# TtesseractT/Synthetic-Audio-Detection

Hardware: AMD Instinct MI355X
Metric: 4s@32kHz segments/sec end-to-end (mel+ResNet+ensemble), 1/2/4/8 MI355X (higher is better)
Workload: dtype bf16; 1 GPU; end-to-end inference: B int16 4 s segments resident in HBM -> mel front end -> ResNet-18@512x512 -> 6 binary heads -> merge (+RCCL all-gather of logits); heads=6, distinct_backbones=1, micro_batch=2048, parallelism=dp1, frontend_overlapped=True

## Files before the change

synthetic-audio-detection_amd/csrc/l2conv.hip:

```cpp
#include "common.hpp"
#include "igemm.hpp"
#include "kernels.hpp"
#include "rwconv.hpp"

namespace sad {

namespace l2c {
constexpr int NW = 4;
constexpr int PW = 18, PR = PW * PW;
constexpr int NDP = (PR + 7) / 8;
constexpr int PATCH = NDP * 1024;
constexpr int ROWB = PW * 128;
constexpr int QP = (NDP + NW - 1) / NW;
constexpr int RESB = 256 * 256;
constexpr int NRP = RESB / 1024 / NW;
constexpr int NDS = 256 * 128 / 1024 / NW;
constexpr int OFF_RES = 2 * PATCH;
constexpr int SMEM_RES = OFF_RES + RESB;
constexpr int NS = 36;
constexpr int NSC = 18;
constexpr int DQ = 4;
constexpr int WV = 8;
constexpr int BAD = 0x7FFFFFF0;
constexpr uint64_t KEY = 0xd92dad912240ull;
constexpr int TABB = NW * QP * 256;
constexpr int TAIL = 512 + TABB;
constexpr int ESH = 27;
static_assert(SMEM_RES + TAIL <= 160 * 1024, "LDS budget");
static_assert(PATCH % 128 == 0 && OFF_RES % 256 == 0, "buffer offsets commute with the chunk XORs");
}

__device__ __forceinline__ int l2c_key(int x) { return (int)((l2c::KEY >> (3 * x)) & 7); }

template <bool RES, bool DS, bool X3, bool ST, bool AB, typename E = u16>
__device__ __forceinline__ void l2conv_body(const BlockConvArgs& a) {
  static_assert(!is_f16_v<E> || (!X3 && !ST && !AB), "fp16: the plain inference forms");
  f16_kernel_entry<E>();
  static_assert(!(RES && DS) && !(X3 && DS), "one shortcut form");
  static_assert(!ST || (!RES && !DS && !X3), "statistics: the plain bf16 form");
  static_assert(!AB || (!X3 && !ST), "ablations: the bf16 forms");
  using namespace l2c;
  constexpr int TP = X3 ? 8 : 16;
  constexpr int UPT = 2 * TP;
  constexpr int NUC = 9 * UPT;
  constexpr int PDIV = X3 ? 8 : 16;
  constexpr int DQ = X3 ? 8 : l2c::DQ;
  constexpr int OFF_B = RES || DS ? SMEM_RES : OFF_RES;
  constexpr int OFF_T = OFF_B + 512;
  extern __shared__ __attribute__((aligned(256))) char smem[];
  const int tid = threadIdx.x, lane = tid & 63;
  const int wave = __builtin_amdgcn_readfirstlane(tid >> 6);
  const int fr = lane & 15, fg = lane >> 4;
  const int ab = AB ? a.ablate : 0;
  const int cw = X3 ? (wave & 1) * 32 : wave * 32;
  const int r0w = X3 ? (wave >> 1) * 8 : 0;
  const int w = xcd_remap(blockIdx.x, gridDim.x);
  const int tiles_x = a.W / 16, tiles_img = tiles_x * (a.H / 16);
  const int tiles_p = a.N * tiles_img;
  const int tp_begin = (int)((int64_t)w * tiles_p / gridDim.x), tp_end = (int)((int64_t)(w + 1) * tiles_p / gridDim.x);
  if (tp_begin >= tp_end) {
    if constexpr (ST) a.st_part[(int64_t)w * 256 + tid] = 0.f;
    return;
  }

  l1b_v4 rx = {(unsigned)(uintptr_t)a.in0, (unsigned)((uintptr_t)a.in0 >> 32) & 0xFFFFu, (unsigned)a.in0_bytes, 0x00020000u};
  asm volatile("" : "+s"(rx));
  const void* const rrp = RES ? (const void*)a.res : (const void*)a.in1;
  l1b_v4 rr = {(unsigned)(uintptr_t)rrp, (unsigned)((uintptr_t)rrp >> 32) & 0xFFFFu,
               (unsigned)(RES ? a.res_bytes : a.in1_bytes), 0x00020000u};
  if constexpr (RES || DS) asm volatile("" : "+s"(rr));
  const __amdgpu_buffer_rsrc_t ro =
      __builtin_amdgcn_make_buffer_rsrc((void*)a.out, (short)0, (int)a.out_bytes, 0x00020000);
  const unsigned lds0 = (unsigned)(uintptr_t)(__attribute__((address_space(3))) char*)smem;
  const int ps = (int)a.in0_pstride * 2;
  const int pso = (int)a.out_pstride * 2;
  const int pss = RES ? (int)a.res_pstride * 2 : DS ? a.ss1 * (int)a.in1_pstride * 2 : 0;
  const int srow = RES ? a.W * pss : DS ? a.ss1 * a.W1 * (int)a.in1_pstride * 2 : 0;
  const int orow = a.W * pso;

  struct TileO {
    int base, oy0, ox0, sbase, obase;
  };
  auto tile_o = [&](int t) __attribute__((always_inline)) {
    const int b = t / tiles_img, rem = t - b * tiles_img;
    const int ty = rem / tiles_x;
    TileO o;
    o.oy0 = ty * 16;
    o.ox0 = (rem - ty * tiles_x) * 16;
    o.base = ((b * a.H + o.oy0) * a.W + o.ox0) * ps;
    o.obase = ((b * a.H + o.oy0) * a.W + o.ox0) * pso;
    o.sbase = RES  ? ((b * a.H + o.oy0) * a.W + o.ox0) * pss
              : DS ? ((b * a.H1 + o.oy0 * a.ss1) * a.W1 + o.ox0 * a.ss1) * (int)(a.in1_pstride * 2)
                   : 0;
    return o;
  };
  const int wrap_i = 15 * a.W * ps, wrap_o = 15 * orow, wrap_s = 16 * srow - a.W * pss;
  auto tile_step = [&](const TileO& o) __attribute__((always_inline)) {
    TileO n;
    n.ox0 = o.ox0 + 16;
    n.oy0 = o.oy0;
    n.base = o.base + 16 * ps;
    n.obase = o.obase + 16 * pso;
    n.sbase = o.sbase + 16 * pss;
    if (n.ox0 == a.W) {
      n.ox0 = 0;
      n.oy0 += 16;
      n.base += wrap_i;
      n.obase += wrap_o;
      n.sbase += wrap_s;
      if (n.oy0 == a.H) n.oy0 = 0;
    }
    return n;
  };

  const int TA = (int)lds0 + OFF_T + (wave * (QP * 64) + lane) * 4;
  auto piece_entry = [&](int k) __attribute__((always_inline)) {
    const int r = 8 * (wave + NW * k) + (lane >> 3);
    const int Y = (r * 3641) >> 16, X = r - PW * Y;
    const int edge = (r >= PR ? 1 : 0) | (Y == 0 ? 2 : 0) | (Y == PW - 1 ? 4 : 0) | (X == 0 ? 8 : 0) | (X == PW - 1 ? 16 : 0);
    const unsigned off = (unsigned)((Y * a.W + X) * ps + (((lane & 7) ^ l2c_key(X)) << 4)) >> 4;
    return (int)(((unsigned)edge << ESH) | (off & ((1u << ESH) - 1)));
  };
  auto patch_base = [&](const TileO& o) __attribute__((always_inline)) { return o.base - (a.W + 1) * ps; };
  auto patch_mask = [&](const TileO& o) __attribute__((always_inline)) {
    return (int)((unsigned)(1 | (o.oy0 == 0 ? 2 : 0) | (o.oy0 + 16 == a.H ? 4 : 0) | (o.ox0 == 0 ? 8 : 0) |
                            (o.ox0 + 16 == a.W ? 16 : 0))
                 << ESH);
  };
  const unsigned dstw = __builtin_amdgcn_readfirstlane(lds0 + wave * 1024);
  auto issue_piece = [&](auto kc, auto cc, int e, int pbase, int pmask) __attribute__((always_inline)) {
    constexpr int k = decltype(kc)::value, c = decltype(cc)::value;
    if constexpr (NW * k + NW - 1 >= NDP)
      if (wave + NW * k >= NDP) return;
    l1b_dma16<c * PATCH + k * NW * 1024>(rx, (e & pmask) ? BAD : pbase + (int)((unsigned)e << 4), dstw);
  };
  const int pxr = 4 * wave + (lane >> 4);
  const int RV = pxr * pss + (((lane & 15) ^ pxr) << 4);
  auto issue_res = [&](auto kc, const TileO& o) __attribute__((always_inline)) {
    constexpr int k = decltype(kc)::value;
    l1b_dma16<OFF_RES + k * NW * 1024>(rr, RV + (o.sbase + k * srow), dstw);
  };
  const int pxd = 8 * (wave & 1) + (lane >> 3);
  const int DV = (wave >> 1) * srow + pxd * pss + (((lane & 7) ^ ((pxd >> 1) & 7)) << 4);
  auto issue_ds = [&](auto kc, const TileO& o) __attribute__((always_inline)) {
    constexpr int k = decltype(kc)::value;
    l1b_dma16<OFF_RES + k * NW * 1024>(rr, DV + (o.sbase + 2 * k * srow), dstw);
  };
  l1b_v4 wds[2][2];
  if constexpr (DS) {
#pragma unroll
    for (int i = 0; i < 2; ++i)
#pragma unroll
      for (int h = 0; h < 2; ++h)
        wds[i][h] = *(const l1b_v4*)((const u16*)a.wt + (size_t)(cw + 16 * i + fr) * a.wt_ld + 9 * 128 + (fg + 4 * h) * 8);
  }

  l1b_v4 wr[2][NS];
#pragma unroll
  for (int i = 0; i < 2; ++i)
#pragma unroll
    for (int s = 0; s < NS; ++s) {
      const int c = s / NSC, tap = (s % NSC) >> 1, h = s & 1;
      wr[i][s] = *(const l1b_v4*)((const u16*)a.wt + (size_t)(cw + 16 * i + fr) * a.wt_ld + tap * 128 + c * 64 +
                                  (fg + 4 * h) * 8);
    }
  if (tid < (X3 ? 16 : 32)) *(float4*)(smem + OFF_B + 16 * tid) = *(const float4*)(a.bias + 4 * tid);
  TileO ocur = tile_o(tp_begin);
  l1b_for<QP>([&](auto kc) __attribute__((always_inline)) {
    constexpr int k = decltype(kc)::value;
    const int e = piece_entry(k);
    l1b_st<int>(TA + 256 * k, e);
    issue_piece(kc, std::integral_constant<int, 0>{}, e, patch_base(ocur), patch_mask(ocur));
  });

  int I2[3];
#pragma unroll
  for (int kx = 0; kx < 3; ++kx)
    I2[kx] = (int)lds0 + r0w * ROWB + (fr + kx) * 128 + ((fg ^ l2c_key(fr + kx)) << 4);
  const int BA = (int)lds0 + OFF_B + (cw + fg * 4) * 4;
  const int OV = ((r0w + (fg & 1)) * a.W + fr) * pso + ((X3 ? 64 * (cw >> 5) : cw) + (fg >> 1) * 8) * 2;
  const int RB = (int)lds0 + OFF_RES + (r0w * 16 + fr) * 256 + ((((X3 ? 8 * (cw >> 5) : cw >> 3) + (fg >> 1)) ^ fr) << 4) +
                 (fg & 1) * 8;
  const int DD = (int)lds0 + OFF_RES + fr * 128 + ((fg ^ ((fr >> 1) & 7)) << 4);
  const int rl = a.relu ? 0 : (int)0x80008000u;
  const bool relu = a.relu;

  asm volatile("s_waitcnt vmcnt(0)" ::: "memory");
  __syncthreads();
  f32x4 acc[2][TP];
#pragma unroll
  for (int i = 0; i < 2; ++i) {
    const f32x4 b0 = l1b_ld<f32x4>(BA + 64 * i);
#pragma unroll
    for (int j = 0; j < TP; ++j) acc[i][j] = b0;
  }

  float st_s[2][4] = {}, st_q[2][4] = {};
  for (int t = tp_begin; t < tp_end; ++t) {
    const TileO ostep = tile_step(ocur);
    const TileO onext = t + 1 < tp_end ? ostep : ocur;
    const TileO o = ocur;
    const int pb1 = patch_base(o) + 128, pm1 = patch_mask(o);
    const int pb0n = patch_base(onext), pm0n = patch_mask(onext);

    l1b_for<2>([&](auto cc) __attribute__((always_inline)) {
      constexpr int c = decltype(cc)::value;
      if constexpr (c == 0)
        asm volatile("s_waitcnt vmcnt(16)" ::: "memory");
      else
        asm volatile("s_waitcnt vmcnt(0)" ::: "memory");
      __builtin_amdgcn_s_barrier();
      asm volatile("" ::: "memory");
      int pe = l1b_ld<int>(TA);
      int I2c[3][2];
#pragma unroll
      for (int kx = 0; kx < 3; ++kx) {
        I2c[kx][0] = I2[kx] + c * PATCH;
        I2c[kx][1] = I2c[kx][0] ^ 64;
      }
      auto rd = [&](auto uc) __attribute__((always_inline)) -> l1b_v4 {
        constexpr int u = decltype(uc)::value;
        constexpr int tap = u / UPT, ky = tap / 3, kx = tap % 3;
        constexpr int j = X3 ? (u % UPT) / 2 : u % 16, h = X3 ? u % 2 : (u % UPT) / 16;
        return l1b_ld<l1b_v4>(I2c[kx][h] + (j + ky) * ROWB);
      };
      l1b_v4 bq[DQ];
      l1b_for<DQ>([&](auto uc) __attribute__((always_inline)) { bq[decltype(uc)::value] = rd(uc); });
      l1b_for<NUC>([&](auto uc) __attribute__((always_inline)) {
        constexpr int u = decltype(uc)::value;
        constexpr int tap = u / UPT;
        constexpr int j = X3 ? (u % UPT) / 2 : u % 16, h = X3 ? u % 2 : (u % UPT) / 16;
        constexpr int s = c * NSC + 2 * tap + h;
        constexpr int s_hi = c * NSC + 2 * tap, s_lo = s_hi + 1;
        const l1b_v4 bf = bq[u % DQ];
        if constexpr (u + DQ < NUC) bq[u % DQ] = rd(std::integral_constant<int, u + DQ>{});
        if constexpr (u % PDIV == 0 && u / PDIV < QP) {
          constexpr int k = u / PDIV;
          if (!(ab & 32))
            issue_piece(std::integral_constant<int, k>{}, std::integral_constant<int, c ^ 1>{}, pe, c == 0 ? pb1 : pb0n,
                        c == 0 ? pm1 : pm0n);
          if constexpr (k + 1 < QP) pe = l1b_ld<int>(TA + 256 * (k + 1));
        }
        if constexpr (RES && c == 0 && u % PDIV == PDIV / 2 && u / PDIV < NRP)
          issue_res(std::integral_constant<int, u / PDIV>{}, o);
        if constexpr (DS && c == 0 && u % 32 == 8 && u / 32 < NDS) issue_ds(std::integral_constant<int, u / 32>{}, o);
        auto mm = [&](auto ic, auto sc) __attribute__((always_inline)) {
          constexpr int i = decltype(ic)::value, ss = decltype(sc)::value;
          if constexpr (i == 1 && ss >= NS - WV)
            l1b_mfma_v<E>(acc[i][j], wr[i][ss], bf);
          else
            l1b_mfma_a<E>(acc[i][j], wr[i][ss], bf);
        };
        if constexpr (!X3) {
          mm(std::integral_constant<int, 0>{}, std::integral_constant<int, s>{});
          mm(std::integral_constant<int, 1>{}, std::integral_constant<int, s>{});
        } else if constexpr (u == NUC - 2) {
          const l1b_v4 xl = bq[(u + 1) % DQ];
          static_assert(j == TP - 1 && h == 0, "last fragment");
          if constexpr (s_hi >= NS - WV)
            asm volatile(
                "v_mfma_f32_16x16x32_bf16 %0, %2, %6, %0\n\t"
                "v_mfma_f32_16x16x32_bf16 %1, %3, %6, %1\n\t"
                "v_mfma_f32_16x16x32_bf16 %0, %4, %6, %0\n\t"
                "v_mfma_f32_16x16x32_bf16 %1, %5, %6, %1\n\t"
                "v_mfma_f32_16x16x32_bf16 %0, %2, %7, %0\n\t"
                "v_mfma_f32_16x16x32_bf16 %1, %3, %7, %1\n\t"
                "s_nop 11"
                : "+v"(acc[0][j]), "+v"(acc[1][j])
                : "a"(wr[0][s_hi]), "v"(wr[1][s_hi]), "a"(wr[0][s_lo]), "v"(wr[1][s_lo]), "v"(bf), "v"(xl));
          else
            asm volatile(
                "v_mfma_f32_16x16x32_bf16 %0, %2, %6, %0\n\t"
                "v_mfma_f32_16x16x32_bf16 %1, %3, %6, %1\n\t"
                "v_mfma_f32_16x16x32_bf16 %0, %4, %6, %0\n\t"
                "v_mfma_f32_16x16x32_bf16 %1, %5, %6, %1\n\t"
                "v_mfma_f32_16x16x32_bf16 %0, %2, %7, %0\n\t"
                "v_mfma_f32_16x16x32_bf16 %1, %3, %7, %1\n\t"
                "s_nop 11"
                : "+v"(acc[0][j]), "+v"(acc[1][j])
                : "a"(wr[0][s_hi]), "a"(wr[1][s_hi]), "a"(wr[0][s_lo]), "a"(wr[1][s_lo]), "v"(bf), "v"(xl));
        } else if constexpr (u == NUC - 1) {
        } else if constexpr (h == 0) {
          mm(std::integral_constant<int, 0>{}, std::integral_constant<int, s_hi>{});
          mm(std::integral_constant<int, 1>{}, std::integral_constant<int, s_hi>{});
          mm(std::integral_constant<int, 0>{}, std::integral_constant<int, s_lo>{});
          mm(std::integral_constant<int, 1>{}, std::integral_constant<int, s_lo>{});
        } else {
          mm(std::integral_constant<int, 0>{}, std::integral_constant<int, s_hi>{});
          mm(std::integral_constant<int, 1>{}, std::integral_constant<int, s_hi>{});
        }
      });
    });
    if constexpr (DS) {
      constexpr int DQD = 8;
      const int DD1 = DD ^ 64;
      auto rdd = [&](auto uc) __attribute__((always_inline)) -> l1b_v4 {
        constexpr int u = decltype(uc)::value;
        return l1b_ld<l1b_v4>((u / 16 ? DD1 : DD) + (u % 16) * 16 * 128);
      };
      l1b_v4 bd[DQD];
      l1b_for<DQD>([&](auto uc) __attribute__((always_inline)) { bd[decltype(uc)::value] = rdd(uc); });
      l1b_for<32>([&](auto uc) __attribute__((always_inline)) {
        constexpr int u = decltype(uc)::value, h = u / 16, j = u % 16;
        const l1b_v4 bf = bd[u % DQD];
        if constexpr (u + DQD < 32) bd[u % DQD] = rdd(std::integral_constant<int, u + DQD>{});
        l1b_mfma_v<E>(acc[0][j], wds[0][h], bf);
        l1b_mfma_v<E>(acc[1][j], wds[1][h], bf);
      });
    }
    __builtin_amdgcn_sched_barrier(0);
    asm volatile("s_nop 11" ::: "memory");
    __builtin_amdgcn_sched_barrier(0);
    f32x4 bv[2];
#pragma unroll
    for (int i = 0; i < 2; ++i) bv[i] = l1b_ld<f32x4>(BA + 64 * i);

#pragma unroll
    for (int j = 0; j < TP; j += 2) {
      const int osj = o.obase + j * orow;
#pragma unroll
      for (int i = 0; i < 2; ++i) {
        f32x4 v0 = acc[i][j], v1 = acc[i][j + 1];
        const int rbi = i ? RB ^ 32 : RB;
        if constexpr (X3) {
          if constexpr (RES) {
            const l1b_v2 h0 = l1b_ld<l1b_v2>(rbi + j * 4096);
            const l1b_v2 l0 = l1b_ld<l1b_v2>((rbi ^ 64) + j * 4096);
            const l1b_v2 h1 = l1b_ld<l1b_v2>(rbi + (j + 1) * 4096);
            const l1b_v2 l1 = l1b_ld<l1b_v2>((rbi ^ 64) + (j + 1) * 4096);
            v0[0] += __uint_as_float(h0.x << 16) + __uint_as_float(l0.x << 16);
            v0[1] += __uint_as_float(h0.x & 0xFFFF0000u) + __uint_as_float(l0.x & 0xFFFF0000u);
            v0[2] += __uint_as_float(h0.y << 16) + __uint_as_float(l0.y << 16);
            v0[3] += __uint_as_float(h0.y & 0xFFFF0000u) + __uint_as_float(l0.y & 0xFFFF0000u);
            v1[0] += __uint_as_float(h1.x << 16) + __uint_as_float(l1.x << 16);
            v1[1] += __uint_as_float(h1.x & 0xFFFF0000u) + __uint_as_float(l1.x & 0xFFFF0000u);
            v1[2] += __uint_as_float(h1.y << 16) + __uint_as_float(l1.y << 16);
            v1[3] += __uint_as_float(h1.y & 0xFFFF0000u) + __uint_as_float(l1.y & 0xFFFF0000u);
          }
          if (relu)
#pragma unroll
            for (int r = 0; r < 4; ++r) {
              v0[r] = fmaxf(v0[r], 0.f);
              v1[r] = fmaxf(v1[r], 0.f);
            }
          uint32_t qh[4] = {l1b_pk(v0[0], v0[1]), l1b_pk(v0[2], v0[3]), l1b_pk(v1[0], v1[1]), l1b_pk(v1[2], v1[3])};
          const float vv[8] = {v0[0], v0[1], v0[2], v0[3], v1[0], v1[1], v1[2], v1[3]};
          uint32_t ql[4];
#pragma unroll
          for (int e = 0; e < 4; ++e)
            ql[e] = l1b_pk(vv[2 * e] - __uint_as_float(qh[e] << 16), vv[2 * e + 1] - __uint_as_float(qh[e] & 0xFFFF0000u));
#pragma unroll
          for (int e = 0; e < 2; ++e) {
            const auto rh = __builtin_amdgcn_permlane16_swap(qh[e], qh[e + 2], false, false);
            qh[e] = rh[0];
            qh[e + 2] = rh[1];
            const auto rl2 = __builtin_amdgcn_permlane16_swap(ql[e], ql[e + 2], false, false);
            ql[e] = rl2[0];
            ql[e + 2] = rl2[1];
          }
          __builtin_amdgcn_raw_buffer_store_b128((l1b_v4){qh[0], qh[1], qh[2], qh[3]}, ro, OV + 32 * i, osj, 0);
          __builtin_amdgcn_raw_buffer_store_b128((l1b_v4){ql[0], ql[1], ql[2], ql[3]}, ro, OV + 32 * i + 64, osj, 0);
          acc[i][j] = bv[i];
          acc[i][j + 1] = bv[i];
          continue;
        }
        if constexpr (RES) {
          const l1b_v2 r0 = l1b_ld<l1b_v2>(rbi + j * 4096);
          const l1b_v2 r1 = l1b_ld<l1b_v2>(rbi + (j + 1) * 4096);
          v0[0] += lo16<E>(r0.x);
          v0[1] += hi16<E>(r0.x);
          v0[2] += lo16<E>(r0.y);
          v0[3] += hi16<E>(r0.y);
          v1[0] += lo16<E>(r1.x);
          v1[1] += hi16<E>(r1.x);
          v1[2] += lo16<E>(r1.y);
          v1[3] += hi16<E>(r1.y);
        }
        if constexpr (ST) {
#pragma unroll
          for (int e = 0; e < 4; ++e) {
            st_s[i][e] += v0[e];
            st_s[i][e] += v1[e];
            st_q[i][e] = fmaf(v0[e], v0[e], st_q[i][e]);
            st_q[i][e] = fmaf(v1[e], v1[e], st_q[i][e]);
          }
        }
        uint32_t q[4] = {l1b_pk<E>(v0[0], v0[1]), l1b_pk<E>(v0[2], v0[3]), l1b_pk<E>(v1[0], v1[1]),
                         l1b_pk<E>(v1[2], v1[3])};
        if constexpr (!ST)
#pragma unroll
          for (int e = 0; e < 4; ++e) q[e] = l1b_relu2s(q[e], rl);
#pragma unroll
        for (int e = 0; e < 2; ++e) {
          const auto r = __builtin_amdgcn_permlane16_swap(q[e], q[e + 2], false, false);
          q[e] = r[0];
          q[e + 2] = r[1];
        }
        if (!(ab & 8)) __builtin_amdgcn_raw_buffer_store_b128((l1b_v4){q[0], q[1], q[2], q[3]}, ro, OV + 32 * i, osj, 0);
        acc[i][j] = bv[i];
        acc[i][j + 1] = bv[i];
      }
    }
    ocur = ostep;
  }
  if constexpr (ST) {
#pragma unroll
    for (int i = 0; i < 2; ++i)
#pragma unroll
      for (int e = 0; e < 4; ++e)
#pragma unroll
        for (int off = 1; off < 16; off <<= 1) {
          st_s[i][e] += __shfl_xor(st_s[i][e], off, 64);
          st_q[i][e] += __shfl_xor(st_q[i][e], off, 64);
        }
    if (fr == 0) {
#pragma unroll
      for (int i = 0; i < 2; ++i)
#pragma unroll
        for (int e = 0; e < 4; ++e) {
          const int c = cw + 16 * i + 4 * fg + e;
          a.st_part[(int64_t)w * 256 + c] = st_s[i][e];
          a.st_part[(int64_t)w * 256 + 128 + c] = st_q[i][e];
        }
    }
  }
  asm volatile("s_waitcnt vmcnt(0)" ::: "memory");
}

template <bool RES, bool DS, bool X3 = false, bool ST = false, typename E = u16>
__global__ __launch_bounds__(256, 1) void l2conv_kernel(BlockConvArgs a) {
  l2conv_body<RES, DS, X3, ST, false, E>(a);
}
template <bool RES, bool DS>
__global__ __launch_bounds__(256, 1) void l2conv_ablate_kernel(BlockConvArgs a) {
  l2conv_body<RES, DS, false, false, true>(a);
}

int launch_l2conv(const BlockConvArgs& a, hipStream_t s, bool x3, bool h16) {
  using namespace l2c;
  SAD_REQUIRE(a.KH == 3 && a.KW == 3 && a.stride == 1 && a.pad == 1 && !a.pool_out,
              "variant 41/42: 3x3/s1/p1, no pool");
  SAD_REQUIRE(!h16 || (!x3 && !a.st_part && !a.ablate), "variant 41 in fp16: the plain inference forms");
  SAD_REQUIRE(!a.st_part || (!x3 && !a.in1 && !a.res && !a.relu && a.st_rows),
              "variant 41 statistics: the plain bf16 raw conv (no shortcut / residual / ReLU), st_rows set");
  if (x3) {
    SAD_REQUIRE(!a.in1 && a.Cin == 128 && a.Cout == 64 && a.H % 16 == 0 && a.W % 16 == 0 && a.Ho == a.H &&
                    a.Wo == a.W && a.wt_ld >= 9 * 128 && a.wt_ld % 8 == 0 && a.in0_pstride % 64 == 0 &&
                    a.in0_pstride >= 128 && a.out_pstride % 64 == 0 && a.out_pstride >= 128 &&
                    (!a.res || (a.res_pstride % 64 == 0 && a.res_pstride >= 128)) && a.out,
                "variant 42: split-bf16 64 -> 64 logical 3x3/s1/p1 (layer1), 16 x 16 tiles");
    const int64_t tiles = (int64_t)a.N * (a.H / 16) * (a.W / 16);
    if (tiles == 0) return SAD_OK;
    const int64_t g = std::min<int64_t>(tiles, 256);
    BlockConvArgs b = a;
    b.out_bytes = ((int64_t)a.N * a.H * a.W - 1) * a.out_pstride * 2 + 256;
    SAD_REQUIRE(b.out_bytes < (1ll << 31) - 65536, "variant 42: output passes the 32-bit buffer range");
    static bool attr[2] = {false, false};
    const void* kfn = a.res ? (const void*)l2conv_kernel<true, false, true> : (const void*)l2conv_kernel<false, false, true>;
    const int smem = (a.res ? SMEM_RES : OFF_RES) + TAIL;
    if (!attr[a.res ? 1 : 0]) {
      SAD_CHECK_HIP(hipFuncSetAttribute(kfn, hipFuncAttributeMaxDynamicSharedMemorySize, smem));
      attr[a.res ? 1 : 0] = true;
    }
    if (a.res)
      hipLaunchKernelGGL((l2conv_kernel<true, false, true>), dim3((unsigned)g), dim3(256), smem, s, b);
    else
      hipLaunchKernelGGL((l2conv_kernel<false, false, true>), dim3((unsigned)g), dim3(256), smem, s, b);
    SAD_CHECK_HIP(hipGetLastError());
    return SAD_OK;
  }
  SAD_REQUIRE(!a.in1 || (!a.res && a.Cin1 == 64 && a.ss1 == 2 && a.H1 == 2 * a.H && a.W1 == 2 * a.W &&
                         a.in1_pstride % 8 == 0 && a.wt_ld >= 9 * 128 + 64),
              "variant 41: the shortcut is a 1x1/2 downsample of a 64-channel input at twice the size");
  SAD_REQUIRE(a.Cin == 128 && a.Cout == 128, "variant 41: Cin = Cout = 128");
  SAD_REQUIRE(a.H % 16 == 0 && a.W % 16 == 0 && a.Ho == a.H && a.Wo == a.W, "variant 41: image must tile by 16 x 16");
  SAD_REQUIRE(a.wt_ld >= 9 * 128 && a.wt_ld % 8 == 0, "variant 41: weight rows");
  SAD_REQUIRE(a.in0_pstride % 8 == 0 && a.out_pstride % 8 == 0 && (!a.res || a.res_pstride % 8 == 0) &&
                  a.in0_pstride >= 128 && a.out_pstride >= 128 && (!a.res || a.res_pstride >= 128),
              "variant 41: 16-B aligned pixel strides");
  SAD_REQUIRE(a.out, "null output");
  const int64_t tiles = (int64_t)a.N * (a.H / 16) * (a.W / 16);
  if (tiles == 0) return SAD_OK;
  const int64_t g = std::min<int64_t>(tiles, 256);
  BlockConvArgs b = a;
  b.out_bytes = ((int64_t)a.N * a.H * a.W - 1) * a.out_pstride * 2 + 256;
  SAD_REQUIRE(b.out_bytes < (1ll << 31) - 65536, "variant 41: output passes the 32-bit buffer range");
  auto go = [&](auto kern, int smem, bool& attr) {
    if (!attr) {
      SAD_CHECK_HIP(hipFuncSetAttribute((const void*)kern, hipFuncAttributeMaxDynamicSharedMemorySize, smem));
      attr = true;
    }
    hipLaunchKernelGGL(kern, dim3((unsigned)g), dim3(256), smem, s, b);
    return SAD_OK;
  };
  static bool attr[10] = {};
  int rc;
  if (h16) {
    rc = a.res   ? go(l2conv_kernel<true, false, false, false, f16>, SMEM_RES + TAIL, attr[7])
         : a.in1 ? go(l2conv_kernel<false, true, false, false, f16>, SMEM_RES + TAIL, attr[8])
                 : go(l2conv_kernel<false, false, false, false, f16>, OFF_RES + TAIL, attr[9]);
  } else if (a.st_part) {
    rc = go(l2conv_kernel<false, false, false, true>, OFF_RES + TAIL, attr[6]);
    if (rc == SAD_OK) *a.st_rows = (int)g;
  } else if (a.res) {
    rc = a.ablate ? go(l2conv_ablate_kernel<true, false>, SMEM_RES + TAIL, attr[3])
                  : go(l2conv_kernel<true, false>, SMEM_RES + TAIL, attr[0]);
  } else if (a.in1) {
    rc = a.ablate ? go(l2conv_ablate_kernel<false, true>, SMEM_RES + TAIL, attr[4])
                  : go(l2conv_kernel<false, true>, SMEM_RES + TAIL, attr[1]);
  } else {
    rc = a.ablate ? go(l2conv_ablate_kernel<false, false>, OFF_RES + TAIL, attr[5])
                  : go(l2conv_kernel<false, false>, OFF_RES + TAIL, attr[2]);
  }
  if (rc != SAD_OK) return rc;
  SAD_CHECK_HIP(hipGetLastError());
  return SAD_OK;
}

}
```

Measured before the change: 64500 segments/s.

## Interleave conv epilogue and downsample MFMAs into the second-half MAC loop

For the non-X3 layer-2 conv, the second chunk's MAC loop is reordered to finish row-pairs early. Each finished pair's epilogue (residual add, stats, pack, relu, permlane swap, store) is then interleaved into the following pair's MFMAs. The downsample 1x1 MFMAs are folded into the same schedule, and the bias is applied through the first MFMA's accumulator input instead of a separate reinit. The aim is to hide the serial epilogue tail behind matrix-core work, at the cost of more complex scheduling and possible extra register pressure.

```diff
diff --git a/synthetic-audio-detection_amd/csrc/l2conv.hip b/synthetic-audio-detection_amd/csrc/l2conv.hip
--- a/synthetic-audio-detection_amd/csrc/l2conv.hip
+++ b/synthetic-audio-detection_amd/csrc/l2conv.hip
@@ -19,6 +19,7 @@
 constexpr int SMEM_RES = OFF_RES + RESB;
 constexpr int NS = 36;
 constexpr int NSC = 18;
+constexpr int SA = 12;
 constexpr int DQ = 4;
 constexpr int WV = 8;
 constexpr int BAD = 0x7FFFFFF0;
@@ -31,6 +32,22 @@
 }
 
 __device__ __forceinline__ int l2c_key(int x) { return (int)((l2c::KEY >> (3 * x)) & 7); }
+
+struct L2Unit {
+  int tap, h, j;
+  bool ds;
+};
+template <bool X3, bool DS>
+constexpr L2Unit l2c_unit(int c, int u) {
+  using l2c::SA;
+  if (X3) return {u / 16, u % 2, (u % 16) / 2, false};
+  if (c == 0 || u < SA * 16) return {u / 32, (u % 32) / 16, u % 16, false};
+  const int nb2 = 2 * (l2c::NSC - SA), upp = nb2 + (DS ? 4 : 0);
+  const int p = (u - SA * 16) / upp, w = (u - SA * 16) % upp;
+  if (w >= nb2) return {0, (w - nb2) / 2, 2 * p + (w - nb2) % 2, true};
+  const int s = SA + w / 2;
+  return {s / 2, s % 2, 2 * p + w % 2, false};
+}
 
 template <bool RES, bool DS, bool X3, bool ST, bool AB, typename E = u16>
 __device__ __forceinline__ void l2conv_body(const BlockConvArgs& a) {
@@ -45,6 +62,15 @@
   constexpr int NUC = 9 * UPT;
   constexpr int PDIV = X3 ? 8 : 16;
   constexpr int DQ = X3 ? 8 : l2c::DQ;
+  constexpr bool FO = !X3;
+  constexpr int NB = NSC - SA;
+  constexpr int UPP = 2 * NB + (DS ? 4 : 0);
+  constexpr int NUA = SA * TP;
+  constexpr int NU1 = FO ? NUA + (TP / 2) * UPP : NUC;
+  constexpr int PD1 = FO ? (NUA / QP < PDIV ? NUA / QP : PDIV) : PDIV;
+  static_assert(!FO || (SA >= 1 && SA < NSC && PD1 >= 1 && PD1 * (QP - 1) < NUA), "phase A carries the 11 pieces");
+  constexpr int EW0 = RES ? 4 : 2, EST = (UPP - EW0) / 8;
+  static_assert(!FO || EST >= 1, "a pair's MFMAs cover the previous pair's epilogue parts");
   constexpr int OFF_B = RES || DS ? SMEM_RES : OFF_RES;
   constexpr int OFF_T = OFF_B + 512;
   extern __shared__ __attribute__((aligned(256))) char smem[];
@@ -188,11 +214,13 @@
   asm volatile("s_waitcnt vmcnt(0)" ::: "memory");
   __syncthreads();
   f32x4 acc[2][TP];
-#pragma unroll
-  for (int i = 0; i < 2; ++i) {
-    const f32x4 b0 = l1b_ld<f32x4>(BA + 64 * i);
-#pragma unroll
-    for (int j = 0; j < TP; ++j) acc[i][j] = b0;
+  if constexpr (!FO) {
+#pragma unroll
+    for (int i = 0; i < 2; ++i) {
+      const f32x4 b0 = l1b_ld<f32x4>(BA + 64 * i);
+#pragma unroll
+      for (int j = 0; j < TP; ++j) acc[i][j] = b0;
+    }
   }
 
   float st_s[2][4] = {}, st_q[2][4] = {};
@@ -202,6 +230,61 @@
     const TileO o = ocur;
     const int pb1 = patch_base(o) + 128, pm1 = patch_mask(o);
     const int pb0n = patch_base(onext), pm0n = patch_mask(onext);
+    f32x4 bv[2];
+    if constexpr (FO) {
+#pragma unroll
+      for (int i = 0; i < 2; ++i) bv[i] = l1b_ld<f32x4>(BA + 64 * i);
+    }
+
+    l1b_v2 er[2][2];
+    uint32_t eq[4];
+    auto epi = [&](auto jc, auto pc) __attribute__((always_inline)) {
+      constexpr int j = decltype(jc)::value, part = decltype(pc)::value;
+      if constexpr (part == 0) {
+        if constexpr (RES) {
+#pragma unroll
+          for (int i = 0; i < 2; ++i)
+#pragma unroll
+            for (int k = 0; k < 2; ++k) er[i][k] = l1b_ld<l1b_v2>((i ? RB ^ 32 : RB) + (j + k) * 4096);
+        }
+      } else {
+        constexpr int i = (part - 1) / 4, k = (part - 1) % 4;
+        if constexpr (k < 2) {
+          f32x4& v = acc[i][j + k];
+          if constexpr (RES) {
+            v[0] += lo16<E>(er[i][k].x);
+            v[1] += hi16<E>(er[i][k].x);
+            v[2] += lo16<E>(er[i][k].y);
+            v[3] += hi16<E>(er[i][k].y);
+          }
+          if constexpr (ST) {
+#pragma unroll
+            for (int e = 0; e < 4; ++e) {
+              st_s[i][e] += v[e];
+              st_q[i][e] = fmaf(v[e], v[e], st_q[i][e]);
+            }
+          }
+        } else if constexpr (k == 2) {
+          const f32x4 v0 = acc[i][j], v1 = acc[i][j + 1];
+          eq[0] = l1b_pk<E>(v0[0], v0[1]);
+          eq[1] = l1b_pk<E>(v0[2], v0[3]);
+          eq[2] = l1b_pk<E>(v1[0], v1[1]);
+          eq[3] = l1b_pk<E>(v1[2], v1[3]);
+          if constexpr (!ST)
+#pragma unroll
+            for (int e = 0; e < 4; ++e) eq[e] = l1b_relu2s(eq[e], rl);
+        } else {
+#pragma unroll
+          for (int e = 0; e < 2; ++e) {
+            const auto r = __builtin_amdgcn_permlane16_swap(eq[e], eq[e + 2], false, false);
+            eq[e] = r[0];
+            eq[e + 2] = r[1];
+          }
+          if (!(ab & 8))
+            __builtin_amdgcn_raw_buffer_store_b128((l1b_v4){eq[0], eq[1], eq[2], eq[3]}, ro, OV + 32 * i, o.obase + j * orow, 0);
+        }
+      }
+    };
 
     l1b_for<2>([&](auto cc) __attribute__((always_inline)) {
       constexpr int c = decltype(cc)::value;
@@ -218,24 +301,28 @@
         I2c[kx][0] = I2[kx] + c * PATCH;
         I2c[kx][1] = I2c[kx][0] ^ 64;
       }
+      constexpr int NU = c == 0 ? NUC : NU1, PD = c == 0 ? PDIV : PD1;
+      const int DD1 = DD ^ 64;
       auto rd = [&](auto uc) __attribute__((always_inline)) -> l1b_v4 {
-        constexpr int u = decltype(uc)::value;
-        constexpr int tap = u / UPT, ky = tap / 3, kx = tap % 3;
-        constexpr int j = X3 ? (u % UPT) / 2 : u % 16, h = X3 ? u % 2 : (u % UPT) / 16;
-        return l1b_ld<l1b_v4>(I2c[kx][h] + (j + ky) * ROWB);
+        constexpr L2Unit U = l2c_unit<X3, DS>(c, decltype(uc)::value);
+        constexpr int ky = U.tap / 3, kx = U.tap % 3;
+        if constexpr (U.ds)
+          return l1b_ld<l1b_v4>((U.h ? DD1 : DD) + U.j * 16 * 128);
+        else
+          return l1b_ld<l1b_v4>(I2c[kx][U.h] + (U.j + ky) * ROWB);
       };
       l1b_v4 bq[DQ];
       l1b_for<DQ>([&](auto uc) __attribute__((always_inline)) { bq[decltype(uc)::value] = rd(uc); });
-      l1b_for<NUC>([&](auto uc) __attribute__((always_inline)) {
+      l1b_for<NU>([&](auto uc) __attribute__((always_inline)) {
         constexpr int u = decltype(uc)::value;
-        constexpr int tap = u / UPT;
-        constexpr int j = X3 ? (u % UPT) / 2 : u % 16, h = X3 ? u % 2 : (u % UPT) / 16;
+        constexpr L2Unit U = l2c_unit<X3, DS>(c, u);
+        constexpr int tap = U.tap, j = U.j, h = U.h;
         constexpr int s = c * NSC + 2 * tap + h;
         constexpr int s_hi = c * NSC + 2 * tap, s_lo = s_hi + 1;
         const l1b_v4 bf = bq[u % DQ];
-        if constexpr (u + DQ < NUC) bq[u % DQ] = rd(std::integral_constant<int, u + DQ>{});
-        if constexpr (u % PDIV == 0 && u / PDIV < QP) {
-          constexpr int k = u / PDIV;
+        if constexpr (u + DQ < NU) bq[u % DQ] = rd(std::integral_constant<int, u + DQ>{});
+        if constexpr (u % PD == 0 && u / PD < QP) {
+          constexpr int k = u / PD;
           if (!(ab & 32))
             issue_piece(std::integral_constant<int, k>{}, std::integral_constant<int, c ^ 1>{}, pe, c == 0 ? pb1 : pb0n,
                         c == 0 ? pm1 : pm0n);
@@ -246,7 +333,11 @@
         if constexpr (DS && c == 0 && u % 32 == 8 && u / 32 < NDS) issue_ds(std::integral_constant<int, u / 32>{}, o);
         auto mm = [&](auto ic, auto sc) __attribute__((always_inline)) {
           constexpr int i = decltype(ic)::value, ss = decltype(sc)::value;
-          if constexpr (i == 1 && ss >= NS - WV)
+          if constexpr (FO && U.ds)
+            l1b_mfma_v<E>(acc[i][j], wds[i][h], bf);
+          else if constexpr (FO && ss == 0)
+            l1b_mfma_ac<E>(acc[i][j], wr[i][ss], bf, bv[i]);
+          else if constexpr (i == 1 && ss >= NS - WV)
             l1b_mfma_v<E>(acc[i][j], wr[i][ss], bf);
           else
             l1b_mfma_a<E>(acc[i][j], wr[i][ss], bf);
@@ -254,6 +345,15 @@
         if constexpr (!X3) {
           mm(std::integral_constant<int, 0>{}, std::integral_constant<int, s>{});
           mm(std::integral_constant<int, 1>{}, std::integral_constant<int, s>{});
+          if constexpr (c == 1 && u >= NUA + UPP) {
+            constexpr int w = (u - NUA) % UPP, jp = 2 * ((u - NUA) / UPP - 1);
+            constexpr int part = w == 0 ? 0 : w >= EW0 && (w - EW0) % EST == 0 && (w - EW0) / EST < 8 ? 1 + (w - EW0) / EST : -1;
+            if constexpr (part == 0 ? RES : part > 0 && (RES || ST || (part - 1) % 4 >= 2)) {
+              __builtin_amdgcn_sched_barrier(0);
+              epi(std::integral_constant<int, jp>{}, std::integral_constant<int, part>{});
+              __builtin_amdgcn_sched_barrier(0);
+            }
+          }
         } else if constexpr (u == NUC - 2) {
           const l1b_v4 xl = bq[(u + 1) % DQ];
           static_assert(j == TP - 1 && h == 0, "last fragment");
@@ -291,38 +391,22 @@
         }
       });
     });
-    if constexpr (DS) {
-      constexpr int DQD = 8;
-      const int DD1 = DD ^ 64;
-      auto rdd = [&](auto uc) __attribute__((always_inline)) -> l1b_v4 {
-        constexpr int u = decltype(uc)::value;
-        return l1b_ld<l1b_v4>((u / 16 ? DD1 : DD) + (u % 16) * 16 * 128);
-      };
-      l1b_v4 bd[DQD];
-      l1b_for<DQD>([&](auto uc) __attribute__((always_inline)) { bd[decltype(uc)::value] = rdd(uc); });
-      l1b_for<32>([&](auto uc) __attribute__((always_inline)) {
-        constexpr int u = decltype(uc)::value, h = u / 16, j = u % 16;
-        const l1b_v4 bf = bd[u % DQD];
-        if constexpr (u + DQD < 32) bd[u % DQD] = rdd(std::integral_constant<int, u + DQD>{});
-        l1b_mfma_v<E>(acc[0][j], wds[0][h], bf);
-        l1b_mfma_v<E>(acc[1][j], wds[1][h], bf);
-      });
-    }
     __builtin_amdgcn_sched_barrier(0);
     asm volatile("s_nop 11" ::: "memory");
     __builtin_amdgcn_sched_barrier(0);
-    f32x4 bv[2];
-#pragma unroll
-    for (int i = 0; i < 2; ++i) bv[i] = l1b_ld<f32x4>(BA + 64 * i);
-
-#pragma unroll
-    for (int j = 0; j < TP; j += 2) {
-      const int osj = o.obase + j * orow;
-#pragma unroll
-      for (int i = 0; i < 2; ++i) {
-        f32x4 v0 = acc[i][j], v1 = acc[i][j + 1];
-        const int rbi = i ? RB ^ 32 : RB;
-        if constexpr (X3) {
+    if constexpr (FO)
+      l1b_for<9>([&](auto pc) __attribute__((always_inline)) { epi(std::integral_constant<int, TP - 2>{}, pc); });
+
+    if constexpr (X3) {
+#pragma unroll
+      for (int i = 0; i < 2; ++i) bv[i] = l1b_ld<f32x4>(BA + 64 * i);
+#pragma unroll
+      for (int j = 0; j < TP; j += 2) {
+        const int osj = o.obase + j * orow;
+#pragma unroll
+        for (int i = 0; i < 2; ++i) {
+          f32x4 v0 = acc[i][j], v1 = acc[i][j + 1];
+          const int rbi = i ? RB ^ 32 : RB;
           if constexpr (RES) {
             const l1b_v2 h0 = l1b_ld<l1b_v2>(rbi + j * 4096);
             const l1b_v2 l0 = l1b_ld<l1b_v2>((rbi ^ 64) + j * 4096);
@@ -362,43 +446,7 @@
           __builtin_amdgcn_raw_buffer_store_b128((l1b_v4){ql[0], ql[1], ql[2], ql[3]}, ro, OV + 32 * i + 64, osj, 0);
           acc[i][j] = bv[i];
           acc[i][j + 1] = bv[i];
-          continue;
-        }
-        if constexpr (RES) {
-          const l1b_v2 r0 = l1b_ld<l1b_v2>(rbi + j * 4096);
-          const l1b_v2 r1 = l1b_ld<l1b_v2>(rbi + (j + 1) * 4096);
-          v0[0] += lo16<E>(r0.x);
-          v0[1] += hi16<E>(r0.x);
-          v0[2] += lo16<E>(r0.y);
-          v0[3] += hi16<E>(r0.y);
-          v1[0] += lo16<E>(r1.x);
-          v1[1] += hi16<E>(r1.x);
-          v1[2] += lo16<E>(r1.y);
-          v1[3] += hi16<E>(r1.y);
-        }
-        if constexpr (ST) {
-#pragma unroll
-          for (int e = 0; e < 4; ++e) {
-            st_s[i][e] += v0[e];
-            st_s[i][e] += v1[e];
-            st_q[i][e] = fmaf(v0[e], v0[e], st_q[i][e]);
-            st_q[i][e] = fmaf(v1[e], v1[e], st_q[i][e]);
-          }
-        }
-        uint32_t q[4] = {l1b_pk<E>(v0[0], v0[1]), l1b_pk<E>(v0[2], v0[3]), l1b_pk<E>(v1[0], v1[1]),
-                         l1b_pk<E>(v1[2], v1[3])};
-        if constexpr (!ST)
-#pragma unroll
-          for (int e = 0; e < 4; ++e) q[e] = l1b_relu2s(q[e], rl);
-#pragma unroll
-        for (int e = 0; e < 2; ++e) {
-          const auto r = __builtin_amdgcn_permlane16_swap(q[e], q[e + 2], false, false);
-          q[e] = r[0];
-          q[e + 2] = r[1];
-        }
-        if (!(ab & 8)) __builtin_amdgcn_raw_buffer_store_b128((l1b_v4){q[0], q[1], q[2], q[3]}, ro, OV + 32 * i, osj, 0);
-        acc[i][j] = bv[i];
-        acc[i][j + 1] = bv[i];
+        }
       }
     }
     ocur = ostep;
```

Result: no change. 64910 segments/s (median of 6 runs) (+0.6%).
